# edwindn/rl-agent-for-qubit-array-tuning

Hardware: AMD Instinct MI355X
Metric: env steps/sec (batched 8-dot 64x64 CSD solves) (higher is better)
Workload: dtype f64; 1 GPU; 8-dot array, 4096 parallel envs per GPU, 64x64 CSD, deterministic physics (latching/noise off), 50-step episodes, staggered phases: 820 episode resets (new device + first observation) inside the timed region, synthetic CNN outputs; n_dots=8, envs_per_gpu=4096, resolution=64

## Files before the change

### rl-agent-for-qubit-array-tuning_amd/csrc/qd_eig.h

```cpp
#pragma once
#include <math.h>
#include "qd_common.h"

#define QD_EIG_REG 12

#if defined(__HIP_DEVICE_COMPILE__)
#define QD_E_ANY(p) (__any((p)) != 0)
QD_HD double qd_rcp(double x) {
    double r = __builtin_amdgcn_rcp(x);
    r = fma(fma(-x, r, 1.0), r, r);
    r = fma(fma(-x, r, 1.0), r, r);
    return r;
}
QD_HD double qd_rcp1(double x) {
    double r = __builtin_amdgcn_rcp(x);
    return fma(fma(-x, r, 1.0), r, r);
}
QD_HD double qd_sqrt1(double x) {
    double y = __builtin_amdgcn_rsq(x);
    y = y * fma(-0.5 * x * y, y, 1.5);
    const double s = x * y;
    return fma(fma(-s, s, x), 0.5 * y, s);
}
QD_HD void qd_sqrt_rsqrt(double x, double& s, double& r) {
// ... 9 lines not shown
QD_HD double qd_rcp(double x) { return 1.0 / x; }
QD_HD double qd_rcp1(double x) { return 1.0 / x; }
QD_HD double qd_sqrt1(double x) { return sqrt(x); }
QD_HD void qd_sqrt_rsqrt(double x, double& s, double& r) { s = sqrt(x); r = 1.0 / s; }
#endif

QD_HD void qd_pow2_scale(double v, double& down, double& up) {
    down = 1.0; up = 1.0;
    union { double d; unsigned long long u; } c; c.d = v;
    const unsigned long long ef = (c.u >> 52) & 0x7FFull;
    if (ef != 0ull && ef < 2046ull) {
        c.u = (2046ull - ef) << 52; down = c.d;
        c.u = ef << 52; up = c.d;
    }
}

QD_HD bool qd_laguerre_step(double dk, double p1, double d1, double e1, double tscale, double& xl) {
    if (p1 == 0.0) return false;
    const double ip = qd_rcp1(p1);
    const double G = d1 * ip, E = e1 * ip;
    const double disc = (dk - 1.0) * ((dk - 1.0) * G * G - dk * E);
    double sq = 0.0;
    if (disc > 0.0) sq = qd_sqrt1(disc);
    const double den = (G < 0.0) ? G - sq : G + sq;
    const double xn = (den != 0.0) ? fma(-dk, qd_rcp1(den), xl) : xl;
    if (!(xn > xl)) return false;
    const double st = xn - xl, tol = 4e-16 * fmax(fmax(fabs(xn), fabs(xl)), 0.05 * tscale);
    xl = xn;
    return st > tol;
}

#define QD_EIG_MAXIT 64

template <int S, bool RESID>
QD_HD void qd_eig_lowest(const double* Ain, double& lam_out, double* x, double& resid_out,
                         int* iters = nullptr, int sz = S) {
    constexpr int NE = S * (S + 1) / 2;
#define QD_IX(i, j) ((i) * ((i) + 1) / 2 + (j))
    double a[NE];
#if defined(__HIP_DEVICE_COMPILE__)
    if (sz == S) {
        const double2* A2 = reinterpret_cast<const double2*>(Ain);
#pragma unroll
        for (int e = 0; e + 1 < NE; e += 2) { const double2 v = A2[e >> 1]; a[e] = v.x; a[e + 1] = v.y; }
        if (NE & 1) a[NE - 1] = Ain[NE - 1];
    } else
#endif
    {
#pragma unroll
        for (int i = 0; i < S; ++i)
#pragma unroll
            for (int j = 0; j <= i; ++j) a[QD_IX(i, j)] = (i < sz) ? Ain[QD_IX(i, j)] : 0.0;
    }
    double anorm = 0.0;
#pragma unroll
    for (int i = 0; i < S; ++i) {
        double rs = 0.0;
#pragma unroll
        for (int j = 0; j < S; ++j) rs += fabs(a[j <= i ? QD_IX(i, j) : QD_IX(j, i)]);
        anorm = fmax(anorm, rs);
    }
    double tsc, tusc;
    qd_pow2_scale(anorm, tsc, tusc);
#pragma unroll
    for (int e = 0; e < NE; ++e) a[e] *= tsc;
#pragma unroll
    for (int i = 0; i < S; ++i) if (i >= sz) a[QD_IX(i, i)] = 4.0;
    double al[S], be[S], tau[S];
#pragma unroll
    for (int k = 0; k + 2 < S; ++k) {
        double sigma = 0.0;
#pragma unroll
        for (int i = k + 2; i < S; ++i) sigma = fma(a[QD_IX(i, k)], a[QD_IX(i, k)], sigma);
        const double x0 = a[QD_IX(k + 1, k)];
        const bool refl = (sigma > 1e-200) & (sigma > 1e-34 * x0 * x0);
        const double mu = qd_sqrt1(fma(x0, x0, sigma) + 1e-300);
        const double v0 = (x0 <= 0.0) ? x0 - mu : -sigma * qd_rcp(x0 + mu);
        const double v0sq = v0 * v0;
        const double t = refl ? 2.0 * v0sq * qd_rcp(sigma + v0sq) : 0.0;
        const double iv0 = refl ? qd_rcp(v0) : 0.0;
#pragma unroll
        for (int i = k + 2; i < S; ++i) a[QD_IX(i, k)] *= iv0;
        tau[k] = t;
        be[k] = refl ? mu : x0;
        al[k] = a[QD_IX(k, k)];
// ... 85 lines not shown
        for (int i = 0; i < S; ++i) y[i] = (i == kbest) ? 1.0 : 0.0;
#pragma unroll
        for (int i = 1; i < S; ++i) if (i > kbest) y[i] = -um[i - 1] * y[i - 1];
#pragma unroll
        for (int i = S - 2; i >= 0; --i) if (i < kbest) y[i] = -lp[i] * y[i + 1];
    }
#pragma unroll
    for (int k = S - 3; k >= 0; --k) {
        double dot = y[k + 1];
#pragma unroll
        for (int i = k + 2; i < S; ++i) dot = fma(a[QD_IX(i, k)], y[i], dot);
        const double f = tau[k] * dot;
        y[k + 1] -= f;
#pragma unroll
        for (int i = k + 2; i < S; ++i) y[i] = fma(-f, a[QD_IX(i, k)], y[i]);
    }
    {
        double nrm = 0.0;
#pragma unroll
        for (int i = 0; i < S; ++i) nrm = fma(y[i], y[i], nrm);
        double sn = 0.0, inv = 1.0;
        if (nrm > 0.0 && nrm < INFINITY) qd_sqrt_rsqrt(nrm, sn, inv);
#pragma unroll
        for (int i = 0; i < S; ++i) y[i] *= inv;
    }
    lam_out = lam * tusc;
    resid_out = 0.0;
    if constexpr (RESID) {
        double r2 = 0.0;
#pragma unroll
        for (int i = 0; i < S; ++i) {
            double acc = -lam_out * y[i];
#pragma unroll
            for (int j = 0; j < S; ++j) if (i < sz && j < sz) acc = fma(Ain[j <= i ? QD_IX(i, j) : QD_IX(j, i)], y[j], acc);
            if (i < sz) r2 = fma(acc, acc, r2);
        }
        resid_out = sqrt(r2);
    }
#pragma unroll
    for (int i = 0; i < S; ++i) x[i] = y[i];
#undef QD_IX
}

QD_HD void qd_eig_lowest_mem(int s, double* M, double* work, const double* Morig,
                             double& lam_out, double& resid_out, int* iters = nullptr) {
#define QD_IX(i, j) ((i) * ((i) + 1) / 2 + (j))
#define QD_SYM(i, j) M[(j) <= (i) ? QD_IX(i, j) : QD_IX(j, i)]
    double* al = work; double* be = work + s; double* tau = work + 2 * s; double* y = work + 3 * s;
    const int ne = s * (s + 1) / 2;
    double anorm = 0.0;
    for (int i = 0; i < s; ++i) {
        double rs = 0.0;
        for (int j = 0; j < s; ++j) rs += fabs(QD_SYM(i, j));
        anorm = fmax(anorm, rs);
    }
    double tsc, tusc;
    qd_pow2_scale(anorm, tsc, tusc);
    for (int e = 0; e < ne; ++e) M[e] *= tsc;
    for (int k = 0; k + 2 < s; ++k) {
        double sigma = 0.0;
        for (int i = k + 2; i < s; ++i) sigma = fma(M[QD_IX(i, k)], M[QD_IX(i, k)], sigma);
        const double x0 = M[QD_IX(k + 1, k)];
        const bool refl = (sigma > 1e-200) & (sigma > 1e-34 * x0 * x0);
        const double mu = qd_sqrt1(fma(x0, x0, sigma) + 1e-300);
        const double v0 = (x0 <= 0.0) ? x0 - mu : -sigma * qd_rcp(x0 + mu);
        const double v0sq = v0 * v0;
        const double t = refl ? 2.0 * v0sq * qd_rcp(sigma + v0sq) : 0.0;
// ... 119 lines not shown
```

### rl-agent-for-qubit-array-tuning_amd/csrc/qd_fullspace.h

```cpp
#pragma once
#include <math.h>
#include <algorithm>
#include "qd_kernels.h"

#define QD_FULL_MAXM 128
#define QD_FULL_MAXSEC 32
#define QD_FULL_MAXNB (2 * (QD_MAXN - 1))

struct QdFullTab {
    int M, nsec, maxsec, pad;
    int sec_start[QD_FULL_MAXSEC + 1];
    int sec[QD_FULL_MAXM];
    unsigned idx[QD_FULL_MAXM];
    unsigned dig[QD_FULL_MAXM];
    int nnb[QD_FULL_MAXM];
    unsigned char nbr[QD_FULL_MAXM][QD_FULL_MAXNB];
    unsigned char nbd[QD_FULL_MAXM][QD_FULL_MAXNB];
    double nbf[QD_FULL_MAXM][QD_FULL_MAXNB];
};

static inline bool qd_full_sizes(int N, int m, int& M, int& maxsec) {
    if (N < 2 || N > QD_MAXN || m < 1) return false;
    M = 1;
    for (int i = 0; i < N; ++i) { M *= m + 1; if (M > QD_FULL_MAXM) return false; }
// ... 26 lines not shown
    for (int q = 0; q < t.nsec; ++q) {
        t.sec_start[q] = p;
        for (int s = 0; s < M; ++s)
            if (charge[s] == q) {
                pos_of[s] = p; t.sec[p] = q; t.idx[p] = (unsigned)s;
                unsigned d = 0;
                for (int i = 0; i < N; ++i) d |= (unsigned)digits[s][i] << (4 * i);
                t.dig[p] = d;
                ++p;
            }
    }
    t.sec_start[t.nsec] = p;
    for (int s = 0; s < M; ++s) {
        const int pi = pos_of[s];
        int k = 0;
        for (int d = 0; d + 1 < N; ++d) {
            const int a = digits[s][d], b = digits[s][d + 1];
            int stride = 1;
            for (int i = d + 2; i < N; ++i) stride *= m + 1;
            if (a >= 1 && b <= m - 1) {
                t.nbr[pi][k] = (unsigned char)pos_of[s - stride * (m + 1) + stride];
                t.nbd[pi][k] = (unsigned char)d; t.nbf[pi][k] = sqrt((double)a * ((double)b + 1.0)); ++k;
            }
            if (b >= 1 && a <= m - 1) {
                t.nbr[pi][k] = (unsigned char)pos_of[s + stride * (m + 1) - stride];
                t.nbd[pi][k] = (unsigned char)d; t.nbf[pi][k] = sqrt((double)b * ((double)a + 1.0)); ++k;
            }
        }
        t.nnb[pi] = k;
    }
}

static inline int qd_full_ppb(const QdFullTab& t, bool validate) {
    size_t pool = 0;
    int tasks[QD_GS_NBIN] = {0};
    for (int q = 0; q < t.nsec; ++q) {
        const int s = t.sec_start[q + 1] - t.sec_start[q];
        if (s >= 2) pool += (size_t)qd_gs_task_doubles(s, validate);
        for (int b = 0; b < QD_GS_NBIN; ++b) tasks[b] += s / qd_gs_bin_min(b);
    }
    size_t ppb = QD_GS_PPB;
    ppb = std::min(ppb, (size_t)(QD_GS_PPB * 32 / t.M));
    if (pool) ppb = std::min(ppb, qd_gs_pool_doubles(validate) / pool);
    for (int b = 0; b < QD_GS_NBIN; ++b)
        if (tasks[b]) ppb = std::min(ppb, (size_t)(qd_gs_list_cap(b) / tasks[b]));
    return ppb < 1 ? 1 : (int)ppb;
}

#if defined(__HIPCC__)

struct QdFullWaveLds {
    double F[QD_FULL_MAXM];
    double lo[QD_FULL_MAXM];
    unsigned long long key[QD_FULL_MAXM];
    unsigned base[QD_FULL_MAXM];
    unsigned gi[QD_FULL_MAXM];
    unsigned char rk[QD_FULL_MAXM];
};

__device__ __forceinline__ double qd_wave_min(double v) {
#pragma unroll
    for (int o = 32; o > 0; o >>= 1) v = fmin(v, __shfl_xor(v, o, 64));
    return v;
}

template <int N>
__device__ __forceinline__ double qd_full_pick(const double* tc, int d) {
    double t = 0.0;
#pragma unroll
    for (int q = 0; q < N - 1; ++q) t = (q == d) ? tc[q] : t;
    return t;
}

template <int N, bool VALIDATE>
__device__ __forceinline__ void qd_full_pixel(const double* __restrict__ par, const double* __restrict__ st, int ch, int R, int p,
                                              int ps, int ppb, const QdFullTab* __restrict__ tab, QdPixelRec* __restrict__ rec,
// ... 50 lines not shown
                }
            }
        }
    }
    const double fshift = qd_wave_min(fmin(F[0], F[1]));
    __builtin_amdgcn_wave_barrier();
#pragma unroll
    for (int h = 0; h < 2; ++h) {
        const int pos = lane + 64 * h;
        if (pos < M) { W.F[pos] = F[h] - fshift; W.lo[pos] = (F[h] - fshift) - rad[h]; W.key[pos] = key[h]; }
    }
    __builtin_amdgcn_wave_barrier();

    int r[2], sz[2], lead[2];
    bool solve[2], active[2];
#pragma unroll
    for (int h = 0; h < 2; ++h) {
        const int pos = lane + 64 * h;
        r[h] = 0; sz[h] = 0; lead[h] = pos; solve[h] = false; active[h] = false;
        if (pos < M) {
            const int q = tab->sec[pos];
            const int s0 = tab->sec_start[q], s1 = tab->sec_start[q + 1];
            double lower = INFINITY;
            for (int j = s0; j < s1; ++j) {
                if (W.key[j] != key[h]) continue;
                if (sz[h] == 0) lead[h] = j;
                r[h] += j < pos ? 1 : 0;
                ++sz[h];
                lower = fmin(lower, W.lo[j]);
            }
            active[h] = lower <= 0.0;
            solve[h] = active[h] && sz[h] > 1;
            W.rk[pos] = (unsigned char)r[h];
            if (solve[h] && r[h] == 0) {
                const unsigned base = atomicAdd(&S.pool_top, (unsigned)qd_gs_task_doubles(sz[h], VALIDATE));
                const int bin = qd_gs_bin(sz[h]);
                const unsigned gi = (unsigned)qd_gs_list_off(bin) + atomicAdd(&S.cnt[bin], 1u);
                sl.lists[gi] = base;
                if (sz[h] > 8) sl.pool[base + 1] = (double)sz[h];
                W.base[pos] = base; W.gi[pos] = gi;
            }
        }
    }
    __builtin_amdgcn_wave_barrier();
    double hn = 0.0;
#pragma unroll
    for (int h = 0; h < 2; ++h) {
        const int pos = lane + 64 * h;
        if (pos >= M) continue;
        if (VALIDATE) hn = fmax(hn, fabs(F[h]) + rad[h]);
        if (!solve[h]) { sl.link[pos * ppb + ps] = active[h] ? QD_LINK_SINGLE : QD_LINK_NONE; sl.rank[pos * ppb + ps] = 0; continue; }
        sl.link[pos * ppb + ps] = W.gi[lead[h]];
        sl.rank[pos * ppb + ps] = (unsigned char)r[h];
        double* row = sl.pool + W.base[lead[h]] + 2 + (r[h] * (r[h] + 1)) / 2;
        for (int c = 0; c < r[h]; ++c) row[c] = 0.0;
        const int nn = tab->nnb[pos];
        for (int k = 0; k < nn; ++k) {
            const double c = -qd_full_pick<N>(tc, tab->nbd[pos][k]) * tab->nbf[pos][k];
            if (c == 0.0) continue;
            const int rj = W.rk[tab->nbr[pos][k]];
            if (rj < r[h]) row[rj] = c;
        }
        row[r[h]] = W.F[pos];
    }
    if (VALIDATE) {
#pragma unroll
        for (int o = 32; o > 0; o >>= 1) hn = fmax(hn, __shfl_xor(hn, o, 64));
        if (lane == 0) { sl.aux[ps] = hn; sl.aux[QD_GS_PPB + ps] = fshift; }
    }
    __builtin_amdgcn_wave_barrier();
}

template <int N, bool VALIDATE>
__global__ void __launch_bounds__(256)
qd_k_full_structure(const int* __restrict__ env_ids, int env_base, int rec_slot0, QdGsGeom g, int ppb, int R,
                    const double* __restrict__ params, const double* __restrict__ state, int noise_flags,
                    const QdFullTab* __restrict__ tab, QdPixelRec* __restrict__ recs, unsigned char* __restrict__ slabs,
                    unsigned* __restrict__ gtiles, unsigned* __restrict__ tilelist, size_t batches_cap) {
    const QdLayout L = qd_layout(N);
    __shared__ QdFullWaveLds sW[4];
    __shared__ QdBlockLds sB;
    const int batch = blockIdx.x;
    const QdSlab sl = qd_gs_slab(slabs + (size_t)batch * qd_gs_slab_bytes(VALIDATE), VALIDATE);
    const int wave = threadIdx.x >> 6;
    const int slot = batch / (g.C * g.nb);
    const int rem = batch - slot * g.C * g.nb;
    const int ch = rem / g.nb, p0 = (rem - ch * g.nb) * ppb;
    const int e = env_ids ? env_ids[env_base + slot] : env_base + slot;
    const double* par = params + (size_t)e * L.size;
    const double* st = state + (size_t)e * L.s_size;
    if (qd_radial_replaced(par, st, L, ch, noise_flags)) {
        if (threadIdx.x < QD_GS_NBIN) sl.cnt[threadIdx.x] = 0;
        return;
    }
    QdPixelRec* rbase = recs + ((size_t)(rec_slot0 + slot) * g.C + ch) * g.P;
    if (threadIdx.x <= QD_GS_NBIN) { if (threadIdx.x == 0) sB.pool_top = 0; else sB.cnt[threadIdx.x - 1] = 0; }
    __syncthreads();
    for (int ps = wave; ps < ppb; ps += 4) {
        const int p = p0 + ps;
        if (p >= g.P) break;
        qd_full_pixel<N, VALIDATE>(par, st, ch, R, p, ps, ppb, tab, rbase + p, sW[wave], sB, sl);
    }
    __syncthreads();
    qd_gs_publish_tiles(sB, sl, batch, gtiles, tilelist, batches_cap);
}

template <int N, bool VALIDATE>
__device__ __forceinline__ void qd_gs_emit(const double* __restrict__ par, const QdLayout& L, const QdPixelRec* __restrict__ rec,
                                           size_t gp, const double* occ, double lam, double resid, double* __restrict__ zraw,
                                           double* __restrict__ occ_out, double* __restrict__ eig_out) {
    constexpr int G = N + 1;
    double b = 0.0;
#pragma unroll
    for (int i = 0; i < N; ++i) b = fma(par[L.cdd_inv + N * G + i], occ[i] - rec->vpp[i], b);
    const double vs = rec->vpp[N];
    const double Ns = rint(vs);
    zraw[gp] = 2.0 * b + par[L.cdd_inv + N * G + N] * (2.0 * (Ns - vs) + 1.0);
    if (occ_out) {
#pragma unroll
        for (int i = 0; i < N; ++i) occ_out[gp * N + i] = occ[i];
    }
    if (VALIDATE && eig_out) { eig_out[gp * 2] = lam; eig_out[gp * 2 + 1] = resid; }
}

template <int N, bool VALIDATE>
__global__ void __launch_bounds__(QD_GS_BLOCK)
qd_k_full_select(const int* __restrict__ env_ids, int env_base, int rec_slot0, QdGsGeom g, int ppb, const double* __restrict__ params,
                 const QdPixelRec* __restrict__ recs, double* __restrict__ zraw, double* __restrict__ occ_out,
                 const double* __restrict__ state, int noise_flags, double* __restrict__ eig_out, const QdFullTab* __restrict__ tab,
                 unsigned char* __restrict__ slabs) {
    const QdLayout L = qd_layout(N);
    const int batch = blockIdx.x;
    const QdSlab sl = qd_gs_slab(slabs + (size_t)batch * qd_gs_slab_bytes(VALIDATE), VALIDATE);
    const int slot = batch / (g.C * g.nb);
    const int rem = batch - slot * g.C * g.nb;
    const int ch = rem / g.nb, p0 = (rem - ch * g.nb) * ppb;
    const int e = env_ids ? env_ids[env_base + slot] : env_base + slot;
    const double* par = params + (size_t)e * L.size;
    const double* st = state + (size_t)e * L.s_size;
    if (qd_radial_replaced(par, st, L, ch, noise_flags)) return;
    const int ps = threadIdx.x, p = p0 + ps;
    if (ps >= ppb || p >= g.P) return;
    const QdPixelRec* rec = recs + ((size_t)(rec_slot0 + slot) * g.C + ch) * g.P + p;
    const int M = tab->M;
    double best = INFINITY; unsigned bestkey = 0xFFFFFFFFu, wl = QD_LINK_NONE; int wpos = 0;
    for (int pos = 0; pos < M; ++pos) {
        const unsigned lk = sl.link[pos * ppb + ps];
        if (lk == QD_LINK_NONE || sl.rank[pos * ppb + ps] != 0) continue;
        const double lam = lk == QD_LINK_SINGLE ? 0.0 : sl.lam[lk];
        const unsigned key = tab->idx[pos];
        if ((lam < best) | ((lam == best) & (key < bestkey))) { best = lam; bestkey = key; wl = lk; wpos = pos; }
    }
    const bool wtask = wl < QD_LINK_SINGLE;
    const unsigned woff = wtask ? sl.lists[wl] : 0u;
    double occ[N];
#pragma unroll
    for (int i = 0; i < N; ++i) occ[i] = 0.0;
    const int q = tab->sec[wpos];
    for (int pos = tab->sec_start[q]; pos < tab->sec_start[q + 1]; ++pos) {
        const bool member = wtask ? sl.link[pos * ppb + ps] == wl : pos == wpos;
        if (!member) continue;
        const double x = wtask ? sl.pool[woff + 2 + sl.rank[pos * ppb + ps]] : 1.0;
        const double pr = x * x;
        const unsigned dg = tab->dig[pos];
#pragma unroll
        for (int i = 0; i < N; ++i) occ[i] = fma(pr, (double)((dg >> (4 * i)) & 15u), occ[i]);
    }
    double lam = best, resid = 0.0;
    if (VALIDATE) {
        const double hn = sl.aux[ps];
        lam = best + sl.aux[QD_GS_PPB + ps];
        if (wtask) resid = sl.pool[woff + 1] / (hn > 0.0 ? hn : 1.0);
    }
    qd_gs_emit<N, VALIDATE>(par, L, rec, ((size_t)e * g.C + ch) * g.P + p, occ, lam, resid, zraw, occ_out, eig_out);
}

#endif
```

### rl-agent-for-qubit-array-tuning_amd/csrc/qd_groundstate.h

```cpp
#pragma once
#include "qd_pixel.h"
#include "qd_eig.h"

#if defined(__HIPCC__)

#ifndef QD_NBREG
#define QD_NBREG 6
#endif
#define QD_GS_BLOCK 256
#define QD_GS_PPB 256
#define QD_GS_NBIN 10
__host__ __device__ inline int qd_gs_bin(int s) { return s <= 8 ? s - 2 : (s <= 10 ? 7 : (s <= 12 ? 8 : 9)); }
__host__ __device__ inline int qd_gs_bin_min(int bin) { return bin <= 6 ? bin + 2 : (bin == 7 ? 9 : (bin == 8 ? 11 : 13)); }
#define QD_LINK_NONE 0xFFFFFFFFu
#define QD_LINK_SINGLE 0xFFFFFFFEu

typedef __attribute__((address_space(3))) double qd_lds_double;
typedef volatile qd_lds_double* qd_lds_vptr;
typedef const volatile qd_lds_double* qd_lds_cvptr;

template <int N>
struct QdWaveLds {
    static constexpr int NS = (2 * (N - 1) - QD_NBREG) > 1 ? (2 * (N - 1) - QD_NBREG) : 1;
    double coef[NS][64];
    unsigned char nidx[NS][64];
    double buf[64];
    double pv[2][16];
    short pfl[2][8];
};
struct QdBlockLds {
    unsigned pool_top;
    unsigned cnt[QD_GS_NBIN];
};

struct QdSlab {
    double* pool; unsigned* link; unsigned char* rank; unsigned* lists; double* aux; unsigned* cnt; double* lam;
};
__host__ __device__ inline int qd_gs_list_cap(int bin) { return QD_GS_PPB * (32 / qd_gs_bin_min(bin)); }
__host__ __device__ inline int qd_gs_list_off(int bin) { int o = 0; for (int b = 0; b < bin; ++b) o += qd_gs_list_cap(b); return o; }
__host__ __device__ inline int qd_gs_task_doubles(int s, bool validate) {
    const int ne = s * (s + 1) / 2;
    const int n = 2 + ne + (s > QD_EIG_REG ? 4 * s + (validate ? ne : 0) : 0);
    return (n + 1) & ~1;
}
__host__ __device__ inline size_t qd_gs_pool_doubles(bool validate) { return (size_t)QD_GS_PPB * (size_t)qd_gs_task_doubles(32, validate); }
__host__ __device__ inline size_t qd_gs_slab_bytes(bool validate) {
    size_t b = qd_gs_pool_doubles(validate) * 8;
    b += (size_t)QD_GS_PPB * 32 * 4;
    b += (size_t)qd_gs_list_off(QD_GS_NBIN) * 4;
    b += (size_t)QD_GS_PPB * 16;
    b += (size_t)QD_GS_PPB * 32;
    b += 64;
    b += (size_t)qd_gs_list_off(QD_GS_NBIN) * 8;
    return (b + 255) & ~(size_t)255;
}
__host__ __device__ inline QdSlab qd_gs_slab(unsigned char* base, bool validate) {
    QdSlab s;
    s.pool = (double*)base; base += qd_gs_pool_doubles(validate) * 8;
    s.link = (unsigned*)base; base += (size_t)QD_GS_PPB * 32 * 4;
    s.lists = (unsigned*)base; base += (size_t)qd_gs_list_off(QD_GS_NBIN) * 4;
    s.aux = (double*)base; base += (size_t)QD_GS_PPB * 16;
    s.rank = base; base += (size_t)QD_GS_PPB * 32;
    s.cnt = (unsigned*)base; base += 64;
    s.lam = (double*)base;
    return s;
}
__host__ __device__ inline size_t qd_gs_tile_cap(int bin, size_t batches) { return batches * (size_t)((qd_gs_list_cap(bin) + 63) / 64); }
__host__ __device__ inline size_t qd_gs_tile_off(int bin, size_t batches) { size_t o = 0; for (int b = 0; b < bin; ++b) o += qd_gs_tile_cap(b, batches); return o; }

__device__ __forceinline__ unsigned qd_half_ballot(bool p) {
    unsigned long long b = __ballot(p);
    return (unsigned)(b >> (threadIdx.x & 32));
}
__device__ __forceinline__ double qd_half_min(double v) {
#pragma unroll
    for (int o = 16; o > 0; o >>= 1) v = fmin(v, __shfl_xor(v, o, 32));
    return v;
}
__device__ __forceinline__ int qd_wave_max_int(int v) {
#pragma unroll
    for (int o = 32; o > 0; o >>= 1) v = max(v, __shfl_xor(v, o, 64));
    return __builtin_amdgcn_readfirstlane(v);
}

template <int N, bool VALIDATE>
__device__ __forceinline__ void qd_ground_structure(const QdPixelRec* __restrict__ rec, bool live, int ps, QdWaveLds<N>& W,
                                                    QdBlockLds& S, const QdSlab& sl, int kept) {
    const int lane = threadIdx.x & 63;
    const int m = lane & 31;
    const int hb = lane & 32;
    const unsigned lt = (1u << m) - 1u;
    qd_lds_vptr buf = (qd_lds_vptr)W.buf;

    const int hh = hb >> 5;
    if (m >= 9 && m < 9 + N - 1) W.pv[hh][m] = rec->tc[m - 9];
    if (m >= 16 && m < 16 + N) W.pfl[hh][m - 16] = (short)rec->fl[m - 16];
    __builtin_amdgcn_wave_barrier();
    const double* pvv = W.pv[hh];
    const bool inK = m < kept;
    const int nvalid = min(rec->nvalid, kept);
    const bool valid = m < nvalid;
    const unsigned code = valid ? (unsigned)rec->idx[m] : 0u;
    unsigned ecode = code;
    ecode = (ecode | (ecode << 8)) & 0x00FF00FFu;
    ecode = (ecode | (ecode << 4)) & 0x0F0F0F0Fu;
    ecode = (ecode | (ecode << 2)) & 0x33333333u;
    const double Fabs = inK ? rec->E[m] : INFINITY;
    const double fshift = qd_half_min(Fabs);
    const double F = Fabs - fshift;

    unsigned tcnz = 0;
#pragma unroll
    for (int d = 0; d < N - 1; ++d) tcnz |= (pvv[9 + d] != 0.0 ? 1u : 0u) << d;
    unsigned tcq = 0;
#pragma unroll
// ... 60 lines not shown
        for (int s = 0; s < maxcnt; ++s) {
            const bool has = rem != 0;
            const int j = has ? __builtin_ctz(rem) : m;
            rem &= rem - 1;
            nw |= __shfl(seg, j, 32);
        }
        const bool changed = nw != seg;
        seg = nw;
        if (!__any(changed)) break;
    }
    const int ssz = __popc(seg);
    const int r = __popc(seg & lt);
    const int smax = qd_wave_max_int(ssz);

    double comp_lower;
    {
        buf[lane] = F - radius;
        __builtin_amdgcn_wave_barrier();
        double acc = INFINITY;
        unsigned mm = seg;
        for (int it = 0; it < smax; ++it) {
            if (mm) { const int b = __builtin_ctz(mm); mm &= mm - 1; acc = fmin(acc, buf[hb + b]); }
        }
        __builtin_amdgcn_wave_barrier();
        comp_lower = acc;
    }
    const bool active = live && comp_lower <= 0.0;
#if defined(QD_ABLATE) && QD_ABLATE == 3
    const bool solve = false;
#else
    const bool solve = active && ssz > 1;
#endif

    unsigned base = 0, gi = 0;
    if (solve && r == 0) {
        base = atomicAdd(&S.pool_top, (unsigned)qd_gs_task_doubles(ssz, VALIDATE));
        const int bin = qd_gs_bin(ssz);
        gi = (unsigned)qd_gs_list_off(bin) + atomicAdd(&S.cnt[bin], 1u);
        sl.lists[gi] = base;
        if (ssz > 8) sl.pool[base + 1] = (double)ssz;
    }
    base = (unsigned)__shfl((int)base, __builtin_ctz(seg), 32);
    gi = (unsigned)__shfl((int)gi, __builtin_ctz(seg), 32);
    if (live) {
        sl.link[ps * 32 + m] = solve ? gi : (active ? QD_LINK_SINGLE : QD_LINK_NONE);
        sl.rank[ps * 32 + m] = (unsigned char)r;
        if (VALIDATE) {
            const double hn = -qd_half_min(inK ? -(fabs(Fabs) + radius) : INFINITY);
            if (m == 0) { sl.aux[ps] = hn; sl.aux[QD_GS_PPB + ps] = fshift; }
        }
    }
    {
        double* row = sl.pool + base + 2 + (r * (r + 1)) / 2;
        unsigned nrm = 0;
        for (int s = 0; s < maxcnt; ++s) {
            if (s < cnt && solve) {
                int j = jreg[0]; double c = creg[0];
                if (s >= QD_NBREG) { j = (int)W.nidx[s - QD_NBREG][lane]; c = W.coef[s - QD_NBREG][lane]; }
#pragma unroll
                for (int i = 1; i < QD_NBREG; ++i) if (i == s) { j = jreg[i]; c = creg[i]; }
                const int rj = __popc(seg & ((1u << j) - 1u));
                if (rj < r) { row[rj] = c; nrm |= 1u << rj; }
            }
        }
        for (int c = 0; c < smax - 1; ++c)
            if (solve && c < r && !((nrm >> c) & 1u)) row[c] = 0.0;
        if (solve) row[r] = F;
    }
}

template <int S, bool PADDED, bool VALIDATE>
__device__ __forceinline__ int qd_eig_task(double* rec, double& lam) {
    double resid, x[S];
    int its = 0;
    const int sz = PADDED ? (int)rec[1] : S;
    qd_eig_lowest<S, VALIDATE>(rec + 2, lam, x, resid, VALIDATE ? &its : nullptr, sz);
    if (VALIDATE) rec[1] = resid;
    if (sz == S) {
        double2* X2 = reinterpret_cast<double2*>(rec + 2);
#pragma unroll
        for (int i = 0; i + 1 < S; i += 2) X2[i >> 1] = make_double2(x[i], x[i + 1]);
        if (S & 1) rec[2 + S - 1] = x[S - 1];
    } else {
#pragma unroll
        for (int i = 0; i < S; ++i) if (i < sz) rec[2 + i] = x[i];
    }
    return its;
}
template <bool VALIDATE>
__device__ __forceinline__ int qd_eig_task_mem(double* rec, double& lam) {
    const int s = (int)rec[1];
    const int ne = s * (s + 1) / 2;
    double* M = rec + 2;
    double* work = M + ne;
    double* copy = VALIDATE ? work + 4 * s : nullptr;
    if (VALIDATE) for (int e = 0; e < ne; ++e) copy[e] = M[e];
    double resid;
    int its = 0;
    qd_eig_lowest_mem(s, M, work, copy, lam, resid, VALIDATE ? &its : nullptr);
    if (VALIDATE) rec[1] = resid;
    for (int i = 0; i < s; ++i) M[i] = work[3 * s + i];
    return its;
}

template <int N, bool VALIDATE, int KC>
__device__ __forceinline__ void qd_ground_select(const QdPixelRec* __restrict__ rec, int ps, const QdSlab& sl,
                                                 double* occ, double& lam_out, double& resid_out) {
    const unsigned* __restrict__ link = sl.link + ps * 32;
    const unsigned char* __restrict__ rank = sl.rank + ps * 32;
    const double* __restrict__ pool = sl.pool;
    const double* __restrict__ lamd = sl.lam;
    const int nvalid = rec->nvalid;
    unsigned lk[KC];
    double lam[KC];
    {
        const uint4* l4 = reinterpret_cast<const uint4*>(link);
#pragma unroll
        for (int q = 0; q < KC / 4; ++q) { const uint4 v = l4[q]; lk[4 * q] = v.x; lk[4 * q + 1] = v.y; lk[4 * q + 2] = v.z; lk[4 * q + 3] = v.w; }
    }
#pragma unroll
    for (int m = 0; m < KC; ++m) {
        const bool task = lk[m] < QD_LINK_SINGLE;
        const double lt = lamd[task ? lk[m] : 0u];
        lam[m] = task ? lt : (lk[m] == QD_LINK_SINGLE ? 0.0 : INFINITY);
    }
    unsigned idx2[KC / 2];
    {
        const uint4* i4 = reinterpret_cast<const uint4*>(rec->idx);
#pragma unroll
        for (int q = 0; q < KC / 8; ++q) { const uint4 v = i4[q]; idx2[4 * q] = v.x; idx2[4 * q + 1] = v.y; idx2[4 * q + 2] = v.z; idx2[4 * q + 3] = v.w; }
    }
    double best = INFINITY; unsigned bestkey = 0xFFFFFFFFu, wl = QD_LINK_NONE; int bm = 0;
#pragma unroll
    for (int m = 0; m < KC; ++m) {
        const unsigned code = (idx2[m >> 1] >> (16 * (m & 1))) & 0xFFFFu;
        const unsigned key = (m < nvalid) ? code : 0xFFFFFFFEu;
        const bool better = (lam[m] < best) | ((lam[m] == best) & (key < bestkey));
        if (better) { best = lam[m]; bestkey = key; wl = lk[m]; bm = m; }
    }
    const bool wtask = wl < QD_LINK_SINGLE;
    const unsigned woff = wtask ? sl.lists[wl] : 0u;
    unsigned rk8[KC / 4];
    {
        if constexpr (KC >= 16) {
            const uint4* r4 = reinterpret_cast<const uint4*>(rank);
#pragma unroll
            for (int q = 0; q < KC / 16; ++q) { const uint4 v = r4[q]; rk8[4 * q] = v.x; rk8[4 * q + 1] = v.y; rk8[4 * q + 2] = v.z; rk8[4 * q + 3] = v.w; }
        } else {
            const uint2 v = *reinterpret_cast<const uint2*>(rank); rk8[0] = v.x; rk8[1] = v.y;
        }
    }
    double xs[KC];
#pragma unroll
    for (int m = 0; m < KC; ++m) {
        const bool member = wtask ? (lk[m] == wl) : (m == bm);
        const unsigned rk = (rk8[m >> 2] >> (8 * (m & 3))) & 0xFFu;
        double x = 0.0;
        if (member) x = wtask ? pool[woff + 2 + rk] : 1.0;
        xs[m] = x;
    }
    int fl[N];
#pragma unroll
    for (int i = 0; i < N; ++i) { occ[i] = 0.0; fl[i] = rec->fl[i]; }
#pragma unroll
    for (int m = 0; m < KC; ++m) {
        const unsigned code = (idx2[m >> 1] >> (16 * (m & 1))) & 0xFFFFu;
        const double p = (m < nvalid) ? xs[m] * xs[m] : 0.0;
#pragma unroll
        for (int i = 0; i < N; ++i)
            occ[i] = fma(p, (double)(fl[i] + (int)((code >> (2 * (N - 1 - i))) & 3u) - 1), occ[i]);
    }
    lam_out = best;
    resid_out = 0.0;
    if (VALIDATE) {
        const double hn = sl.aux[ps];
        lam_out = best + sl.aux[QD_GS_PPB + ps];
        if (wtask) resid_out = pool[woff + 1] / (hn > 0.0 ? hn : 1.0);
    }
}

#endif
```

### rl-agent-for-qubit-array-tuning_amd/csrc/qd_kernels.h

```cpp
#pragma once
#include "qd_groundstate.h"
#include "qd_rng.h"

#if defined(__HIPCC__)

struct QdRewardCfg {
    double gate_ramp_start, gate_quadratic_start, barrier_ramp_start;
    int max_steps;
    int use_deltas, sparse, curve;
    double delta_max, curve_exponent;
    double plunger_radius, outer_plunger_radius, outer_plunger_reward_max, barrier_radius;
};

__device__ __forceinline__ double qd_gate_reward(double dist, const QdRewardCfg& rc) {
    if (rc.sparse) {
        if (dist <= rc.plunger_radius) return 1.0;
        if (dist <= rc.outer_plunger_radius) {
            const double nd = (dist - rc.plunger_radius) / (rc.outer_plunger_radius - rc.plunger_radius);
            return rc.outer_plunger_reward_max * (1.0 - nd);
        }
        return 0.0;
    }
    double r;
    if (dist >= rc.gate_ramp_start) r = 0.0;
// ... 202 lines not shown
                tl[t] = ((unsigned)batch << 12) | (t << 6) | (here - 1u);
            }
        }
    }
}

#ifndef QD_GS_WAVES
#define QD_GS_WAVES 7
#endif
template <int N, bool VALIDATE, int WPB>
__global__ void __launch_bounds__(64 * WPB, WPB == 4 ? QD_GS_WAVES : 4)
qd_k_gs_structure(const int* __restrict__ env_ids, int env_base, int rec_slot0, QdGsGeom g, int R, const double* __restrict__ params,
                  const QdPixelRec* __restrict__ recs, const double* __restrict__ state, int noise_flags,
                  unsigned char* __restrict__ slabs, unsigned* __restrict__ gtiles, unsigned* __restrict__ tilelist, size_t batches_cap,
                  int kept) {
    const QdLayout L = qd_layout(N);
    __shared__ QdWaveLds<N> sW[WPB];
    __shared__ QdBlockLds sB;
    constexpr int PPW = QD_GS_PPB / WPB;
    const int batch = blockIdx.x;
    const QdSlab sl = qd_gs_slab(slabs + (size_t)batch * qd_gs_slab_bytes(VALIDATE), VALIDATE);
    const int wave = threadIdx.x >> 6, lane = threadIdx.x & 63;
    int slot, ch, p0;
    qd_gs_locate(g, batch, slot, ch, p0);
    const int e = env_ids ? env_ids[env_base + slot] : env_base + slot;
    const double* par = params + (size_t)e * L.size;
    const double* st = state + (size_t)e * L.s_size;
    if (qd_radial_replaced(par, st, L, ch, noise_flags)) {
        if (threadIdx.x < QD_GS_NBIN) sl.cnt[threadIdx.x] = 0;
        return;
    }
    const QdPixelRec* rbase = recs + ((size_t)(rec_slot0 + slot) * g.C + ch) * g.P;
    if (threadIdx.x <= QD_GS_NBIN) { if (threadIdx.x == 0) sB.pool_top = 0; else sB.cnt[threadIdx.x - 1] = 0; }
    __syncthreads();
    QdWaveLds<N>& W = sW[wave];
    for (int it = 0; it < PPW / 2; ++it) {
        const int ps = wave * PPW + it * 2 + (lane >> 5);
        if (p0 + wave * PPW + it * 2 >= g.P) break;
        const int p = p0 + ps;
        const int pc = p < g.P ? p : g.P - 1;
        qd_ground_structure<N, VALIDATE>(rbase + pc, p < g.P, ps, W, sB, sl, kept);
    }
    __syncthreads();
    qd_gs_publish_tiles(sB, sl, batch, gtiles, tilelist, batches_cap);
}

template <int BIN, bool VALIDATE>
__device__ __forceinline__ int qd_gs_solve_task(double* rec, double& lam) {
    if constexpr (BIN <= 6) return qd_eig_task<BIN + 2, false, VALIDATE>(rec, lam);
    else if constexpr (BIN == 7) return qd_eig_task<10, true, VALIDATE>(rec, lam);
    else if constexpr (BIN == 8) return qd_eig_task<12, true, VALIDATE>(rec, lam);
    else return qd_eig_task_mem<VALIDATE>(rec, lam);
}
template <int BIN> struct QdGsSolveWaves { static constexpr int v = BIN <= 1 ? 6 : (BIN == 2 ? 4 : (BIN == 3 ? 3 : (BIN <= 6 ? 2 : (BIN == 9 ? 4 : 1)))); };

template <int BIN, bool VALIDATE>
__global__ void __launch_bounds__(256, QdGsSolveWaves<BIN>::v)
qd_k_gs_solve(unsigned char* __restrict__ slabs, const unsigned* __restrict__ gtiles, const unsigned* __restrict__ tilelist,
              size_t batches_cap, unsigned long long* __restrict__ stats) {
    const int lane = threadIdx.x & 63;
    const unsigned ntile = gtiles[BIN];
    const unsigned* tl = tilelist + qd_gs_tile_off(BIN, batches_cap);
    const unsigned nwaves = gridDim.x * 4u;
    unsigned gt = blockIdx.x * 4u + (threadIdx.x >> 6);
    const size_t slab_bytes = qd_gs_slab_bytes(VALIDATE);
    auto offset_of = [&](unsigned d) -> unsigned {
        const QdSlab sl = qd_gs_slab(slabs + (size_t)(d >> 12) * slab_bytes, VALIDATE);
        return lane <= (int)(d & 63u) ? sl.lists[qd_gs_list_off(BIN) + (int)((d >> 6) & 63u) * 64 + lane] : 0u;
    };
    unsigned desc = gt < ntile ? tl[gt] : 0u;
    unsigned desc1 = gt + nwaves < ntile ? tl[gt + nwaves] : 0u;
    unsigned off = gt < ntile ? offset_of(desc) : 0u;
    for (; gt < ntile; gt += nwaves) {
        const unsigned desc2 = gt + 2u * nwaves < ntile ? tl[gt + 2u * nwaves] : 0u;
        const unsigned off1 = gt + nwaves < ntile ? offset_of(desc1) : 0u;
        const unsigned batch = desc >> 12;
        const int here = (int)(desc & 63u) + 1;
        const QdSlab sl = qd_gs_slab(slabs + (size_t)batch * slab_bytes, VALIDATE);
        int its = 0;
        if (lane < here) {
            double lam;
            its = qd_gs_solve_task<BIN, VALIDATE>(sl.pool + off, lam);
            sl.lam[qd_gs_list_off(BIN) + (int)((desc >> 6) & 63u) * 64 + lane] = lam;
        }
        desc = desc1; desc1 = desc2; off = off1;
        if (VALIDATE && stats) {
            int sum = its, mx = its;
#pragma unroll
            for (int o = 32; o > 0; o >>= 1) { sum += __shfl_xor(sum, o, 64); mx = max(mx, __shfl_xor(mx, o, 64)); }
            if (lane == 0) {
                atomicAdd(&stats[16], (unsigned long long)here); atomicAdd(&stats[17], (unsigned long long)sum);
                atomicAdd(&stats[18], 1ull); atomicAdd(&stats[19], (unsigned long long)mx);
                atomicAdd(&stats[20 + BIN], (unsigned long long)here);
            }
        }
    }
}

#ifndef QD_SEL_WAVES
#define QD_SEL_WAVES 3
#endif
template <int N, bool VALIDATE, int KC>
__global__ void __launch_bounds__(QD_GS_BLOCK, QD_SEL_WAVES)
qd_k_gs_select(const int* __restrict__ env_ids, int env_base, int rec_slot0, QdGsGeom g, int R, const double* __restrict__ params,
               const QdPixelRec* __restrict__ recs, double* __restrict__ zraw, double* __restrict__ occ_out,
               const double* __restrict__ state, int noise_flags, double* __restrict__ eig_out, unsigned char* __restrict__ slabs) {
    constexpr int G = N + 1;
// ... 566 lines not shown
```

Measured before the change: 12600 env-steps/s.

## Interleave small eigen-task matrices across 64-task tiles for coalesced solver loads

Tasks in bins below 9 (sizes up to 12) are now allocated in tiles of 64 slots, with each task's packed matrix stored at stride 64. Adjacent lanes of a solve wave therefore read consecutive doubles, replacing per-lane strided record reads. The first task in each tile reserves the tile's pool space and publishes its base in LDS, and other tasks spin-wait on that entry. Pool sizing gains a per-bin tile-waste allowance and a worst-case split bound, and the solve kernel reads descriptors as scalars via readfirstlane. The cost is extra pool padding, LDS state, and a spin-wait in the builder.

```diff
diff --git a/rl-agent-for-qubit-array-tuning_amd/csrc/qd_eig.h b/rl-agent-for-qubit-array-tuning_amd/csrc/qd_eig.h
--- a/rl-agent-for-qubit-array-tuning_amd/csrc/qd_eig.h
+++ b/rl-agent-for-qubit-array-tuning_amd/csrc/qd_eig.h
@@ -65,14 +65,14 @@
 
 #define QD_EIG_MAXIT 64
 
-template <int S, bool RESID>
+template <int S, bool RESID, int ST = 1>
 QD_HD void qd_eig_lowest(const double* Ain, double& lam_out, double* x, double& resid_out,
                          int* iters = nullptr, int sz = S) {
     constexpr int NE = S * (S + 1) / 2;
 #define QD_IX(i, j) ((i) * ((i) + 1) / 2 + (j))
     double a[NE];
 #if defined(__HIP_DEVICE_COMPILE__)
-    if (sz == S) {
+    if (ST == 1 && sz == S) {
         const double2* A2 = reinterpret_cast<const double2*>(Ain);
 #pragma unroll
         for (int e = 0; e + 1 < NE; e += 2) { const double2 v = A2[e >> 1]; a[e] = v.x; a[e + 1] = v.y; }
@@ -83,7 +83,7 @@
 #pragma unroll
         for (int i = 0; i < S; ++i)
 #pragma unroll
-            for (int j = 0; j <= i; ++j) a[QD_IX(i, j)] = (i < sz) ? Ain[QD_IX(i, j)] : 0.0;
+            for (int j = 0; j <= i; ++j) a[QD_IX(i, j)] = (i < sz) ? Ain[QD_IX(i, j) * ST] : 0.0;
     }
     double anorm = 0.0;
 #pragma unroll
@@ -235,7 +235,7 @@
         for (int i = 0; i < S; ++i) {
             double acc = -lam_out * y[i];
 #pragma unroll
-            for (int j = 0; j < S; ++j) if (i < sz && j < sz) acc = fma(Ain[j <= i ? QD_IX(i, j) : QD_IX(j, i)], y[j], acc);
+            for (int j = 0; j < S; ++j) if (i < sz && j < sz) acc = fma(Ain[(j <= i ? QD_IX(i, j) : QD_IX(j, i)) * ST], y[j], acc);
             if (i < sz) r2 = fma(acc, acc, r2);
         }
         resid_out = sqrt(r2);
diff --git a/rl-agent-for-qubit-array-tuning_amd/csrc/qd_fullspace.h b/rl-agent-for-qubit-array-tuning_amd/csrc/qd_fullspace.h
--- a/rl-agent-for-qubit-array-tuning_amd/csrc/qd_fullspace.h
+++ b/rl-agent-for-qubit-array-tuning_amd/csrc/qd_fullspace.h
@@ -82,16 +82,24 @@
 }
 
 static inline int qd_full_ppb(const QdFullTab& t, bool validate) {
+    size_t worst[QD_K + 1] = {0};
+    for (int s = 2; s <= QD_K; ++s) {
+        worst[s] = (size_t)qd_gs_cost_doubles(s, validate);
+        for (int a = 1; a < s; ++a) worst[s] = std::max(worst[s], worst[a] + worst[s - a]);
+    }
     size_t pool = 0;
     int tasks[QD_GS_NBIN] = {0};
     for (int q = 0; q < t.nsec; ++q) {
         const int s = t.sec_start[q + 1] - t.sec_start[q];
-        if (s >= 2) pool += (size_t)qd_gs_task_doubles(s, validate);
+        pool += worst[s];
         for (int b = 0; b < QD_GS_NBIN; ++b) tasks[b] += s / qd_gs_bin_min(b);
     }
+    size_t waste = 0;
+    for (int b = 0; b < QD_GS_TILED; ++b)
+        if (tasks[b]) waste += 63 * (size_t)qd_gs_slot_doubles(b);
     size_t ppb = QD_GS_PPB;
     ppb = std::min(ppb, (size_t)(QD_GS_PPB * 32 / t.M));
-    if (pool) ppb = std::min(ppb, qd_gs_pool_doubles(validate) / pool);
+    if (pool) ppb = std::min(ppb, (qd_gs_pool_doubles(validate) - waste) / pool);
     for (int b = 0; b < QD_GS_NBIN; ++b)
         if (tasks[b]) ppb = std::min(ppb, (size_t)(qd_gs_list_cap(b) / tasks[b]));
     return ppb < 1 ? 1 : (int)ppb;
@@ -208,15 +216,11 @@
             active[h] = lower <= 0.0;
             solve[h] = active[h] && sz[h] > 1;
             W.rk[pos] = (unsigned char)r[h];
-            if (solve[h] && r[h] == 0) {
-                const unsigned base = atomicAdd(&S.pool_top, (unsigned)qd_gs_task_doubles(sz[h], VALIDATE));
-                const int bin = qd_gs_bin(sz[h]);
-                const unsigned gi = (unsigned)qd_gs_list_off(bin) + atomicAdd(&S.cnt[bin], 1u);
-                sl.lists[gi] = base;
-                if (sz[h] > 8) sl.pool[base + 1] = (double)sz[h];
-                W.base[pos] = base; W.gi[pos] = gi;
-            }
         }
+        unsigned gi, base;
+        int sh;
+        qd_gs_new_task<VALIDATE>(S, sl, solve[h] && r[h] == 0, sz[h], gi, base, sh);
+        if (solve[h] && r[h] == 0) { W.base[pos] = base; W.gi[pos] = gi; }
     }
     __builtin_amdgcn_wave_barrier();
     double hn = 0.0;
@@ -228,16 +232,17 @@
         if (!solve[h]) { sl.link[pos * ppb + ps] = active[h] ? QD_LINK_SINGLE : QD_LINK_NONE; sl.rank[pos * ppb + ps] = 0; continue; }
         sl.link[pos * ppb + ps] = W.gi[lead[h]];
         sl.rank[pos * ppb + ps] = (unsigned char)r[h];
-        double* row = sl.pool + W.base[lead[h]] + 2 + (r[h] * (r[h] + 1)) / 2;
-        for (int c = 0; c < r[h]; ++c) row[c] = 0.0;
+        const int sh = qd_gs_bin(sz[h]) < QD_GS_TILED ? QD_GS_ILG : 0;
+        double* row = sl.pool + W.base[lead[h]] + ((2 + (r[h] * (r[h] + 1)) / 2) << sh);
+        for (int c = 0; c < r[h]; ++c) row[c << sh] = 0.0;
         const int nn = tab->nnb[pos];
         for (int k = 0; k < nn; ++k) {
             const double c = -qd_full_pick<N>(tc, tab->nbd[pos][k]) * tab->nbf[pos][k];
             if (c == 0.0) continue;
             const int rj = W.rk[tab->nbr[pos][k]];
-            if (rj < r[h]) row[rj] = c;
+            if (rj < r[h]) row[rj << sh] = c;
         }
-        row[r[h]] = W.F[pos];
+        row[r[h] << sh] = W.F[pos];
     }
     if (VALIDATE) {
 #pragma unroll
@@ -271,6 +276,7 @@
     }
     QdPixelRec* rbase = recs + ((size_t)(rec_slot0 + slot) * g.C + ch) * g.P;
     if (threadIdx.x <= QD_GS_NBIN) { if (threadIdx.x == 0) sB.pool_top = 0; else sB.cnt[threadIdx.x - 1] = 0; }
+    for (int t = threadIdx.x; t < QD_GS_NTILE_TILED; t += 256) sB.tbase[t] = QD_TBASE_NONE;
     __syncthreads();
     for (int ps = wave; ps < ppb; ps += 4) {
         const int p = p0 + ps;
@@ -328,7 +334,9 @@
         if ((lam < best) | ((lam == best) & (key < bestkey))) { best = lam; bestkey = key; wl = lk; wpos = pos; }
     }
     const bool wtask = wl < QD_LINK_SINGLE;
-    const unsigned woff = wtask ? sl.lists[wl] : 0u;
+    unsigned woff = 0u;
+    int wsh = 0;
+    if (wtask) qd_gs_task_rec(sl, wl, woff, wsh);
     double occ[N];
 #pragma unroll
     for (int i = 0; i < N; ++i) occ[i] = 0.0;
@@ -336,7 +344,7 @@
     for (int pos = tab->sec_start[q]; pos < tab->sec_start[q + 1]; ++pos) {
         const bool member = wtask ? sl.link[pos * ppb + ps] == wl : pos == wpos;
         if (!member) continue;
-        const double x = wtask ? sl.pool[woff + 2 + sl.rank[pos * ppb + ps]] : 1.0;
+        const double x = wtask ? sl.pool[woff + ((2u + sl.rank[pos * ppb + ps]) << wsh)] : 1.0;
         const double pr = x * x;
         const unsigned dg = tab->dig[pos];
 #pragma unroll
@@ -346,7 +354,7 @@
     if (VALIDATE) {
         const double hn = sl.aux[ps];
         lam = best + sl.aux[QD_GS_PPB + ps];
-        if (wtask) resid = sl.pool[woff + 1] / (hn > 0.0 ? hn : 1.0);
+        if (wtask) resid = sl.pool[woff + (1u << wsh)] / (hn > 0.0 ? hn : 1.0);
     }
     qd_gs_emit<N, VALIDATE>(par, L, rec, ((size_t)e * g.C + ch) * g.P + p, occ, lam, resid, zraw, occ_out, eig_out);
 }
diff --git a/rl-agent-for-qubit-array-tuning_amd/csrc/qd_groundstate.h b/rl-agent-for-qubit-array-tuning_amd/csrc/qd_groundstate.h
--- a/rl-agent-for-qubit-array-tuning_amd/csrc/qd_groundstate.h
+++ b/rl-agent-for-qubit-array-tuning_amd/csrc/qd_groundstate.h
@@ -28,22 +28,46 @@
     double pv[2][16];
     short pfl[2][8];
 };
+#define QD_GS_TILED 9
+#define QD_GS_ILG 6
+#define QD_GS_IL (1 << QD_GS_ILG)
+__host__ __device__ inline int qd_gs_bin_max(int bin) { return bin <= 6 ? bin + 2 : (bin == 7 ? 10 : (bin == 8 ? 12 : 32)); }
+__host__ __device__ inline int qd_gs_list_cap(int bin) { return QD_GS_PPB * (32 / qd_gs_bin_min(bin)); }
+__host__ __device__ inline int qd_gs_list_off(int bin) { int o = 0; for (int b = 0; b < bin; ++b) o += qd_gs_list_cap(b); return o; }
+#define QD_GS_NTILE_TILED (QD_GS_PPB * 58 / 64)
+static_assert(QD_GS_NTILE_TILED * 64 == QD_GS_PPB * (16 + 10 + 8 + 6 + 5 + 4 + 4 + 3 + 2), "tile table of the tiled classes");
+#define QD_TBASE_NONE 0xFFFFFFFFu
 struct QdBlockLds {
     unsigned pool_top;
     unsigned cnt[QD_GS_NBIN];
+    unsigned tbase[QD_GS_NTILE_TILED];
 };
+typedef __attribute__((address_space(3))) unsigned qd_lds_uint;
 
 struct QdSlab {
     double* pool; unsigned* link; unsigned char* rank; unsigned* lists; double* aux; unsigned* cnt; double* lam;
 };
-__host__ __device__ inline int qd_gs_list_cap(int bin) { return QD_GS_PPB * (32 / qd_gs_bin_min(bin)); }
-__host__ __device__ inline int qd_gs_list_off(int bin) { int o = 0; for (int b = 0; b < bin; ++b) o += qd_gs_list_cap(b); return o; }
 __host__ __device__ inline int qd_gs_task_doubles(int s, bool validate) {
     const int ne = s * (s + 1) / 2;
     const int n = 2 + ne + (s > QD_EIG_REG ? 4 * s + (validate ? ne : 0) : 0);
     return (n + 1) & ~1;
 }
-__host__ __device__ inline size_t qd_gs_pool_doubles(bool validate) { return (size_t)QD_GS_PPB * (size_t)qd_gs_task_doubles(32, validate); }
+__host__ __device__ inline int qd_gs_slot_doubles(int bin) { const int s = qd_gs_bin_max(bin); return 2 + s * (s + 1) / 2; }
+__host__ __device__ inline unsigned qd_gs_slot_off(int bin, unsigned t) {
+    return (t >> QD_GS_ILG) * (unsigned)(QD_GS_IL * qd_gs_slot_doubles(bin)) + (t & (QD_GS_IL - 1u));
+}
+__host__ __device__ inline int qd_gs_cost_doubles(int s, bool validate) {
+    const int bin = qd_gs_bin(s);
+    return bin < QD_GS_TILED ? qd_gs_slot_doubles(bin) : qd_gs_task_doubles(s, validate);
+}
+__host__ __device__ inline size_t qd_gs_tile_waste_doubles() {
+    size_t w = 0;
+    for (int b = 0; b < QD_GS_TILED; ++b) w += 63 * (size_t)qd_gs_slot_doubles(b);
+    return w;
+}
+__host__ __device__ inline size_t qd_gs_pool_doubles(bool validate) {
+    return (size_t)QD_GS_PPB * (size_t)qd_gs_task_doubles(32, validate) + qd_gs_tile_waste_doubles();
+}
 __host__ __device__ inline size_t qd_gs_slab_bytes(bool validate) {
     size_t b = qd_gs_pool_doubles(validate) * 8;
     b += (size_t)QD_GS_PPB * 32 * 4;
@@ -81,6 +105,40 @@
 #pragma unroll
     for (int o = 32; o > 0; o >>= 1) v = max(v, __shfl_xor(v, o, 64));
     return __builtin_amdgcn_readfirstlane(v);
+}
+
+template <bool VALIDATE>
+__device__ __forceinline__ void qd_gs_new_task(QdBlockLds& S, const QdSlab& sl, bool want, int s, unsigned& gi, unsigned& rb, int& sh) {
+    volatile qd_lds_uint* tbase = (volatile qd_lds_uint*)S.tbase;
+    const int bin = qd_gs_bin(s);
+    const bool tiled = bin < QD_GS_TILED;
+    gi = 0; rb = 0; sh = tiled ? QD_GS_ILG : 0;
+    if (want) {
+        gi = (unsigned)qd_gs_list_off(bin) + atomicAdd(&S.cnt[bin], 1u);
+        if (!tiled) {
+            rb = atomicAdd(&S.pool_top, (unsigned)qd_gs_task_doubles(s, VALIDATE));
+            sl.lists[gi] = rb;
+        } else if ((gi & 63u) == 0u) {
+            rb = atomicAdd(&S.pool_top, 64u * (unsigned)qd_gs_slot_doubles(bin));
+            sl.lists[gi] = rb;
+            tbase[gi >> 6] = rb;
+        }
+    }
+    if (want && tiled && (gi & 63u) != 0u) {
+        unsigned v = tbase[gi >> 6];
+        for (int g = 0; v == QD_TBASE_NONE && g < (1 << 24); ++g) { __builtin_amdgcn_s_sleep(1); v = tbase[gi >> 6]; }
+        rb = v;
+    }
+    if (want && tiled) rb += qd_gs_slot_off(bin, gi & 63u);
+    if (want && s > 8) sl.pool[rb + (1u << sh)] = (double)s;
+}
+__device__ __forceinline__ void qd_gs_task_rec(const QdSlab& sl, unsigned gi, unsigned& rb, int& sh) {
+    const bool tiled = gi < (unsigned)qd_gs_list_off(QD_GS_TILED);
+    int bin = 0;
+#pragma unroll
+    for (int b = 1; b < QD_GS_TILED; ++b) bin += gi >= (unsigned)qd_gs_list_off(b) ? 1 : 0;
+    rb = tiled ? sl.lists[gi & ~63u] + qd_gs_slot_off(bin, gi & 63u) : sl.lists[gi];
+    sh = tiled ? QD_GS_ILG : 0;
 }
 
 template <int N, bool VALIDATE>
@@ -207,14 +265,9 @@
     const bool solve = active && ssz > 1;
 #endif
 
-    unsigned base = 0, gi = 0;
-    if (solve && r == 0) {
-        base = atomicAdd(&S.pool_top, (unsigned)qd_gs_task_doubles(ssz, VALIDATE));
-        const int bin = qd_gs_bin(ssz);
-        gi = (unsigned)qd_gs_list_off(bin) + atomicAdd(&S.cnt[bin], 1u);
-        sl.lists[gi] = base;
-        if (ssz > 8) sl.pool[base + 1] = (double)ssz;
-    }
+    unsigned base, gi;
+    int sh;
+    qd_gs_new_task<VALIDATE>(S, sl, solve && r == 0, ssz, gi, base, sh);
     base = (unsigned)__shfl((int)base, __builtin_ctz(seg), 32);
     gi = (unsigned)__shfl((int)gi, __builtin_ctz(seg), 32);
     if (live) {
@@ -226,7 +279,7 @@
         }
     }
     {
-        double* row = sl.pool + base + 2 + (r * (r + 1)) / 2;
+        double* row = sl.pool + base + ((2 + (r * (r + 1)) / 2) << sh);
         unsigned nrm = 0;
         for (int s = 0; s < maxcnt; ++s) {
             if (s < cnt && solve) {
@@ -235,23 +288,26 @@
 #pragma unroll
                 for (int i = 1; i < QD_NBREG; ++i) if (i == s) { j = jreg[i]; c = creg[i]; }
                 const int rj = __popc(seg & ((1u << j) - 1u));
-                if (rj < r) { row[rj] = c; nrm |= 1u << rj; }
+                if (rj < r) { row[rj << sh] = c; nrm |= 1u << rj; }
             }
         }
         for (int c = 0; c < smax - 1; ++c)
-            if (solve && c < r && !((nrm >> c) & 1u)) row[c] = 0.0;
-        if (solve) row[r] = F;
-    }
-}
-
-template <int S, bool PADDED, bool VALIDATE>
+            if (solve && c < r && !((nrm >> c) & 1u)) row[c << sh] = 0.0;
+        if (solve) row[r << sh] = F;
+    }
+}
+
+template <int S, bool PADDED, bool VALIDATE, int ST = 1>
 __device__ __forceinline__ int qd_eig_task(double* rec, double& lam) {
     double resid, x[S];
     int its = 0;
-    const int sz = PADDED ? (int)rec[1] : S;
-    qd_eig_lowest<S, VALIDATE>(rec + 2, lam, x, resid, VALIDATE ? &its : nullptr, sz);
-    if (VALIDATE) rec[1] = resid;
-    if (sz == S) {
+    const int sz = PADDED ? (int)rec[ST] : S;
+    qd_eig_lowest<S, VALIDATE, ST>(rec + 2 * ST, lam, x, resid, VALIDATE ? &its : nullptr, sz);
+    if (VALIDATE) rec[ST] = resid;
+    if (ST > 1) {
+#pragma unroll
+        for (int i = 0; i < S; ++i) if (i < sz) rec[(2 + i) * ST] = x[i];
+    } else if (sz == S) {
         double2* X2 = reinterpret_cast<double2*>(rec + 2);
 #pragma unroll
         for (int i = 0; i + 1 < S; i += 2) X2[i >> 1] = make_double2(x[i], x[i + 1]);
@@ -314,7 +370,9 @@
         if (better) { best = lam[m]; bestkey = key; wl = lk[m]; bm = m; }
     }
     const bool wtask = wl < QD_LINK_SINGLE;
-    const unsigned woff = wtask ? sl.lists[wl] : 0u;
+    unsigned woff = 0u;
+    int wsh = 0;
+    if (wtask) qd_gs_task_rec(sl, wl, woff, wsh);
     unsigned rk8[KC / 4];
     {
         if constexpr (KC >= 16) {
@@ -331,7 +389,7 @@
         const bool member = wtask ? (lk[m] == wl) : (m == bm);
         const unsigned rk = (rk8[m >> 2] >> (8 * (m & 3))) & 0xFFu;
         double x = 0.0;
-        if (member) x = wtask ? pool[woff + 2 + rk] : 1.0;
+        if (member) x = wtask ? pool[woff + ((2 + rk) << wsh)] : 1.0;
         xs[m] = x;
     }
     int fl[N];
@@ -350,7 +408,7 @@
     if (VALIDATE) {
         const double hn = sl.aux[ps];
         lam_out = best + sl.aux[QD_GS_PPB + ps];
-        if (wtask) resid_out = pool[woff + 1] / (hn > 0.0 ? hn : 1.0);
+        if (wtask) resid_out = pool[woff + (1u << wsh)] / (hn > 0.0 ? hn : 1.0);
     }
 }
 
diff --git a/rl-agent-for-qubit-array-tuning_amd/csrc/qd_kernels.h b/rl-agent-for-qubit-array-tuning_amd/csrc/qd_kernels.h
--- a/rl-agent-for-qubit-array-tuning_amd/csrc/qd_kernels.h
+++ b/rl-agent-for-qubit-array-tuning_amd/csrc/qd_kernels.h
@@ -258,6 +258,7 @@
     }
     const QdPixelRec* rbase = recs + ((size_t)(rec_slot0 + slot) * g.C + ch) * g.P;
     if (threadIdx.x <= QD_GS_NBIN) { if (threadIdx.x == 0) sB.pool_top = 0; else sB.cnt[threadIdx.x - 1] = 0; }
+    for (int t = threadIdx.x; t < QD_GS_NTILE_TILED; t += 64 * WPB) sB.tbase[t] = QD_TBASE_NONE;
     __syncthreads();
     QdWaveLds<N>& W = sW[wave];
     for (int it = 0; it < PPW / 2; ++it) {
@@ -273,9 +274,9 @@
 
 template <int BIN, bool VALIDATE>
 __device__ __forceinline__ int qd_gs_solve_task(double* rec, double& lam) {
-    if constexpr (BIN <= 6) return qd_eig_task<BIN + 2, false, VALIDATE>(rec, lam);
-    else if constexpr (BIN == 7) return qd_eig_task<10, true, VALIDATE>(rec, lam);
-    else if constexpr (BIN == 8) return qd_eig_task<12, true, VALIDATE>(rec, lam);
+    if constexpr (BIN <= 6) return qd_eig_task<BIN + 2, false, VALIDATE, QD_GS_IL>(rec, lam);
+    else if constexpr (BIN == 7) return qd_eig_task<10, true, VALIDATE, QD_GS_IL>(rec, lam);
+    else if constexpr (BIN == 8) return qd_eig_task<12, true, VALIDATE, QD_GS_IL>(rec, lam);
     else return qd_eig_task_mem<VALIDATE>(rec, lam);
 }
 template <int BIN> struct QdGsSolveWaves { static constexpr int v = BIN <= 1 ? 6 : (BIN == 2 ? 4 : (BIN == 3 ? 3 : (BIN <= 6 ? 2 : (BIN == 9 ? 4 : 1)))); };
@@ -292,13 +293,17 @@
     const size_t slab_bytes = qd_gs_slab_bytes(VALIDATE);
     auto offset_of = [&](unsigned d) -> unsigned {
         const QdSlab sl = qd_gs_slab(slabs + (size_t)(d >> 12) * slab_bytes, VALIDATE);
-        return lane <= (int)(d & 63u) ? sl.lists[qd_gs_list_off(BIN) + (int)((d >> 6) & 63u) * 64 + lane] : 0u;
+        const unsigned* lp = sl.lists + qd_gs_list_off(BIN) + (int)((d >> 6) & 63u) * 64;
+        if constexpr (BIN < QD_GS_TILED) return (unsigned)__builtin_amdgcn_readfirstlane((int)lp[0]) + qd_gs_slot_off(BIN, (unsigned)lane);
+        else return lane <= (int)(d & 63u) ? lp[lane] : 0u;
     };
-    unsigned desc = gt < ntile ? tl[gt] : 0u;
-    unsigned desc1 = gt + nwaves < ntile ? tl[gt + nwaves] : 0u;
+    auto desc_at = [&](unsigned i) -> unsigned { return (unsigned)__builtin_amdgcn_readfirstlane((int)tl[i]); };
+    gt = (unsigned)__builtin_amdgcn_readfirstlane((int)gt);
+    unsigned desc = gt < ntile ? desc_at(gt) : 0u;
+    unsigned desc1 = gt + nwaves < ntile ? desc_at(gt + nwaves) : 0u;
     unsigned off = gt < ntile ? offset_of(desc) : 0u;
     for (; gt < ntile; gt += nwaves) {
-        const unsigned desc2 = gt + 2u * nwaves < ntile ? tl[gt + 2u * nwaves] : 0u;
+        const unsigned desc2 = gt + 2u * nwaves < ntile ? desc_at(gt + 2u * nwaves) : 0u;
         const unsigned off1 = gt + nwaves < ntile ? offset_of(desc1) : 0u;
         const unsigned batch = desc >> 12;
         const int here = (int)(desc & 63u) + 1;
```

Measured after the change: 12740 env-steps/s (median of 6 runs). Within noise of the previous version (+1.1%).
